# gabrielmpp/LagrangianCoherence

Hardware: AMD Instinct MI355X
Metric: particle-timesteps/sec (+ FTLE Mcells/sec) at 4096^2 seeds per GPU (higher is better)
Workload: dtype f32

## Files before the change

### include/lcs_hip.h

```cpp
#ifndef LCS_HIP_H
#define LCS_HIP_H

#include <stddef.h>
#include <stdint.h>

#ifdef __cplusplus
extern "C" {
#endif

#define LC_VERSION 104

typedef struct lc_ctx lc_ctx;

enum lc_dtype {
    LC_F32 = 0,
    LC_F64 = 1,
    LC_F64_WIND_F32 = 2,
    LC_F64_WIND_F32_LIN32 = 3
};

enum lc_status {
    LC_OK = 0,
    LC_EINVAL = -1,
    LC_EUNSUPPORTED = -2,
// ... 11 lines not shown
enum lc_tensor_layout {
    LC_LAYOUT_REFERENCE = 0,
    LC_LAYOUT_PHYSICAL = 1
};

int lc_version(void);
const char *lc_last_error(void);
const char *lc_build_id(void);

int lc_ctx_create(int device, lc_ctx **out);
int lc_ctx_destroy(lc_ctx *ctx);
int lc_ctx_set_stream(lc_ctx *ctx, void *hip_stream );
int lc_ctx_use_own_stream(lc_ctx *ctx);
int lc_sync(lc_ctx *ctx);

int lc_ctx_set_lds_tiles(lc_ctx *ctx, int mode);
int lc_ctx_set_sigma_march(lc_ctx *ctx, int on);
typedef int (*lc_flag_allreduce_fn)(void *user, void *flags_dev, size_t count);
int lc_ctx_set_flag_allreduce(lc_ctx *ctx, lc_flag_allreduce_fn fn, void *user);
int lc_ctx_set_level_chunk(lc_ctx *ctx, int levels);
int lc_ctx_get_level_chunk(const lc_ctx *ctx, int *levels_out);
int lc_ctx_set_level_grading(lc_ctx *ctx, int chunk, int zone, int depth);
int lc_ctx_get_level_grading(const lc_ctx *ctx, int *chunk_out, int *zone_out, int *depth_out);
enum lc_f64_fidelity { LC_F64_AUTO = 0, LC_F64_EXACT_ORDER = 1, LC_F64_FAST = 2 };
#define LC_EXACT_ORDER_MAX_SEEDS (1 << 18)
int lc_ctx_set_f64_fidelity(lc_ctx *ctx, int mode);
int lc_ctx_get_f64_fidelity(const lc_ctx *ctx, int *mode_out);
int lc_ctx_set_host_pipeline(lc_ctx *ctx, int on);
int lc_copy_to_device(lc_ctx *ctx, void *dst_dev, const void *src_host, size_t bytes);
int lc_copy_to_host(lc_ctx *ctx, void *dst_host, const void *src_dev, size_t bytes);
int lc_ctx_set_host_cache(lc_ctx *ctx, int on);
int lc_ctx_trim(lc_ctx *ctx);
int lc_ctx_last_host_marks(const lc_ctx *ctx, double *ms4_out);
int lc_ctx_set_xcd_split(lc_ctx *ctx, int split);
const char *lc_ctx_last_advect_kernel(const lc_ctx *ctx);
int lc_ctx_last_advect_launches(const lc_ctx *ctx);
const char *lc_ctx_last_sigma_kernel(const lc_ctx *ctx);
const char *lc_ctx_last_pack_kernel(const lc_ctx *ctx);
const char *lc_ctx_last_tracer_kernel(const lc_ctx *ctx);
#define LC_VERIFY_WORDS 16
int lc_ctx_set_verify(lc_ctx *ctx, int mode);
int lc_ctx_read_verify(lc_ctx *ctx, unsigned *out16, int reset);

int lc_malloc(lc_ctx *ctx, size_t bytes, void **dev_out);
int lc_free(lc_ctx *ctx, void *dev);
int lc_memcpy_h2d(lc_ctx *ctx, void *dev_dst, const void *host_src, size_t bytes);
// ... 196 lines not shown
```

### lagrangiancoherence_amd/_capi.py

```python
from __future__ import annotations

import ctypes as C
import os

HERE = os.path.dirname(os.path.abspath(__file__))
LIB_PATH = os.path.join(HERE, "liblcs_hip.so")

LC_VERSION = 104
LC_F32, LC_F64, LC_F64_WIND_F32, LC_F64_WIND_F32_LIN32 = 0, 1, 2, 3
LC_OK, LC_EINVAL, LC_EUNSUPPORTED, LC_EHIP, LC_ENOMEM, LC_ERCCL = 0, -1, -2, -3, -4, -5
LC_LAYOUT_REFERENCE, LC_LAYOUT_PHYSICAL = 0, 1
LC_X_CLAMP_POINT, LC_X_CYCLIC, LC_X_CLAMP_REFERENCE_OUTER = 0, 1, 2
LC_GRID_REGULAR, LC_GRID_GAUSSIAN = 0, 1
LC_F64_AUTO, LC_F64_EXACT_ORDER, LC_F64_FAST = 0, 1, 2
LC_EXACT_ORDER_MAX_SEEDS = 1 << 18

_vp, _i, _d, _sz = C.c_void_p, C.c_int, C.c_double, C.c_size_t

PROTOTYPES = {
    "lc_version": (_i, []),
    "lc_last_error": (C.c_char_p, []),
    "lc_build_id": (C.c_char_p, []),
    "lc_ctx_create": (_i, [_i, C.POINTER(_vp)]),
    "lc_ctx_destroy": (_i, [_vp]),
    "lc_ctx_set_stream": (_i, [_vp, _vp]),
    "lc_ctx_use_own_stream": (_i, [_vp]),
    "lc_sync": (_i, [_vp]),
    "lc_ctx_set_lds_tiles": (_i, [_vp, _i]),
    "lc_ctx_set_sigma_march": (_i, [_vp, _i]),
    "lc_ctx_set_level_chunk": (_i, [_vp, _i]),
    "lc_ctx_get_level_chunk": (_i, [_vp, C.POINTER(_i)]),
    "lc_ctx_set_level_grading": (_i, [_vp, _i, _i, _i]),
    "lc_ctx_get_level_grading": (_i, [_vp, C.POINTER(_i), C.POINTER(_i), C.POINTER(_i)]),
    "lc_ctx_set_f64_fidelity": (_i, [_vp, _i]),
    "lc_ctx_get_f64_fidelity": (_i, [_vp, C.POINTER(_i)]),
    "lc_ctx_set_host_pipeline": (_i, [_vp, _i]),
    "lc_ctx_last_host_marks": (_i, [_vp, C.POINTER(C.c_double)]),
    "lc_copy_to_device": (_i, [_vp, _vp, _vp, C.c_size_t]),
    "lc_copy_to_host": (_i, [_vp, _vp, _vp, C.c_size_t]),
    "lc_ctx_set_host_cache": (_i, [_vp, _i]),
    "lc_ctx_trim": (_i, [_vp]),
    "lc_ctx_set_xcd_split": (_i, [_vp, _i]),
    "lc_ctx_set_flag_allreduce": (_i, [_vp, _vp, _vp]),
    "lc_ctx_last_advect_kernel": (C.c_char_p, [_vp]),
    "lc_ctx_last_advect_launches": (_i, [_vp]),
    "lc_ctx_last_sigma_kernel": (C.c_char_p, [_vp]),
    "lc_ctx_last_pack_kernel": (C.c_char_p, [_vp]),
    "lc_ctx_last_tracer_kernel": (C.c_char_p, [_vp]),
    "lc_ctx_set_verify": (_i, [_vp, _i]),
    "lc_ctx_read_verify": (_i, [_vp, C.POINTER(C.c_uint), _i]),
    "lc_malloc": (_i, [_vp, _sz, C.POINTER(_vp)]),
    "lc_free": (_i, [_vp, _vp]),
    "lc_memcpy_h2d": (_i, [_vp, _vp, _vp, _sz]),
    "lc_memcpy_d2h": (_i, [_vp, _vp, _vp, _sz]),
    "lc_packed_elems": (_sz, [_i, _i, _i]),
    "lc_field_pack": (_i, [_vp, _vp, _vp, _i, _i, _i, _i, _i, _vp, _vp]),
# ... 147 lines not shown
```

### lagrangiancoherence_amd/csrc/advect.hip

```cpp
#include <initializer_list>
#include <type_traits>
#include <vector>

#include "lcs_common.h"
#include "launch_plan.h"

namespace {

constexpr int TILE_W = 8;
constexpr int TILE_H = 32;
constexpr int BLOCK = TILE_W * TILE_H;

template <typename T>
struct AdvectArgs {
    const T *lin;
    const T *img;
    const T *ext;
    const T *u_raw, *v_raw;
    const float *lin32;
    const float *u_raw32, *v_raw32;
    size_t raw_plane;
    int ext_raw;
    int ext_cub;
    size_t level_elems;
// ... 14 lines not shown
    int n_members, member_t0_stride;
    size_t member_plane;
    int pair_d, pair_l0, pair_n, pair_g, pair_last;
    size_t pair_plane;
    int traj_skip0;
    int traj_pair_ok, out_pair_ok;
    int traj_line_ok;
    int patch_mode;
    int xcd_rows;
    int xcd_split;
    int wg64;
    int ntx, ntiles;
    int xcd_chunk;
    int tile_order;
    int tile_order_two_seed;
    int pole_blocks, pole_lo, pole_hi;
    unsigned *clamp_flag;
    int clamp_stride;
    unsigned *verify;
    int member_dirs;
    lcplan::Grading grade;
    int grade_launch, grade_t0;
    const T *grade_x_start, *grade_y_start;
#ifdef LCS_TIMELINE
    unsigned long long *timeline;
    int timeline_launch;
#endif
};

template <typename T>
__device__ __forceinline__ int xcd_tile_id(const AdvectArgs<T> &A) {
    return lcplan::tile_of_block((int)blockIdx.x - A.pole_blocks, A.ntiles, A.ntx, A.xcd_chunk, A.tile_order);
}
template <typename T>
static inline unsigned nmem(const AdvectArgs<T> &A) { return A.n_members > 1 ? (unsigned)A.n_members : 1u; }

template <typename K, typename T, typename... Extra>
static inline const char *launch_kernel(K kernel, int grid, hipStream_t st, const AdvectArgs<T> &A, const char *name, const Extra &...extra) {
    hipLaunchKernelGGL(kernel, dim3(grid, nmem(A)), dim3(BLOCK), 0, st, A, extra...);
    return name;
}

template <typename T>
struct Instance {
    int K;
    bool cyclic;
// ... 1472 lines not shown
#endif
#ifndef LCS_LDS2_DPP_NEXT
#define LCS_LDS2_DPP_NEXT 1
#endif
#ifndef LCS_LDS2_DIRECT_LEVELS
#define LCS_LDS2_DIRECT_LEVELS 0
#endif
template <int KFIX, bool CYCLIC, int MODE>
__global__ void __launch_bounds__(BLOCK, LCS_LDS2_MINWAVES) __attribute__((amdgpu_num_sgpr(LCS_LDS2_NUM_SGPR)))
    advect_lds2_kernel(const AdvectArgs<float> A0) {
#pragma clang fp contract(fast)
    const AdvectArgs<float> A = for_member(A0);
    constexpr bool WIDE = MODE == PATCH_WIDE, LINES = MODE == PATCH_LINES, GROUP = MODE == PATCH_PAIR;
    constexpr int NS = SPL;
    constexpr int ORDER = 1;
    constexpr bool DEFER_X = LCS_LDS2_DEFER_X != 0;
    constexpr int DIRECT_LEVELS = DEFER_X ? LCS_LDS2_DIRECT_LEVELS : 0;
    constexpr bool DPP_NEXT = LCS_LDS2_DPP_NEXT != 0 && 16 % Lds2Geom::LANES_PER_ROW == 0;
    const int K = KFIX >= 0 ? KFIX : A.K;
    typedef Lds2Geom G;
    constexpr int LT_COLS = G::COLS, LT_ROWS = LCS_LDS2_ROWS;
    constexpr int LT_PITCH = LCS_LDS2_PITCH;
    constexpr int WIN = 2, WOFF = LC_PAD_LO;
    __shared__ __attribute__((aligned(16))) f4 s_tiles[BLOCK / 64][LT_ROWS * LT_PITCH];
    __shared__ __attribute__((aligned(16))) float s_slab[2][2][LINES ? 16 * SLAB_PITCH : 4];
    if (GROUP ? pole_block_group(A) : pole_block<float, POLE_LIN>(A)) return;
    int tile_id, t0 = A.t0, nsteps = A.nsteps;
    const float *x_from = A.x_start, *y_from = A.y_start;
    if (MODE == PATCH_TALL && A.grade.n > 0) {
        const int d = (int)blockIdx.x - A.pole_blocks;
        tile_id = lcplan::tile_of_block(lcplan::graded_slot(A.grade, A.grade_launch, d), A.ntiles, A.ntx, A.xcd_chunk, A.tile_order);
        if (tile_id >= A.ntiles) return;
        const lcplan::Range r = lcplan::graded_range(A.grade, A.grade_launch, d);
        if (r.b <= r.a) return;
        t0 = A.grade_t0 + r.a;
        nsteps = r.b - r.a;
        x_from = r.a == 0 ? A.grade_x_start : A.x_out;
        y_from = r.a == 0 ? A.grade_y_start : A.y_out;
    } else {
        tile_id = xcd_tile_id(A);
        if (tile_id >= A.ntiles) return;
    }
    const int tyi = tile_id / A.ntx, txi = tile_id - tyi * A.ntx;
    const int lane = threadIdx.x & 63, wave = threadIdx.x >> 6;
#ifdef LCS_TIMELINE
    unsigned long long *const tl_rec = A.timeline ? A.timeline + ((size_t)A.timeline_launch * gridDim.x + blockIdx.x) * 4 : nullptr;
    if (tl_rec && threadIdx.x == 0) {
// ... 74 lines not shown
    unsigned pitch_bytes = (unsigned)LT_PITCH * 16u;
    asm volatile("" : "+s"(pitch_bytes));
    const f2 pmin = {A.lon_min, A.lat_min}, sc = {A.sx, A.sy};
    auto to_index = [&](f2 v) { return (v - pmin) * sc; };
    const float xlo = A.x_min, xhi = A.x_max;
    auto x_needs_care = [&](float x) { return CYCLIC ? !(fabsf(x) < 180.0f) : !((x > xlo) & (x < xhi)); };
    const float *lvl = A.img + (size_t)t0 * A.level_elems;
    const float *elv = A.ext + (size_t)t0 * A.level_elems;
    const int pad_cols = A.pitch, pad_rows = A.ny_f + LC_PAD;
    const float kpred = 0.5f * (float)(K > 0 ? K - 1 : 0);
    const int st_row = min(lane / G::LANES_PER_ROW, LT_ROWS - 1), st_col = (lane % G::LANES_PER_ROW) * 2;
    const unsigned st_off = ((unsigned)st_row * (unsigned)pad_cols + (unsigned)st_col) * 8u;
    constexpr int NPASS = (LT_ROWS + G::ROWS_PER_PASS - 1) / G::ROWS_PER_PASS;
    const unsigned st_next = st_off + (st_col + 2 < LT_COLS ? 16u : 0u);
    constexpr int CENTRE = (WIDE || GROUP) ? TILE_W / 2 + TILE_W * 4 : TILE_W / 2 + TILE_W * 7;
    f2 dprev = {0.0f, 0.0f};
    const int nlev = GROUP ? lcplan::group_levels(A.nsteps, A.pair_l0, A.pair_n, A.pair_d, cnt) : nsteps;
#ifdef LCS_STAMPS
    long long acc_t[5] = {0, 0, 0, 0, 0}, last_t = __builtin_amdgcn_s_memtime();
    unsigned long long acc_n[3] = {0, 0, 0};
    int prev_redos = 0;
#endif
    int direct_left = 0;
    for (int s = 0; s < nlev; ++s) {
        const bool direct = DIRECT_LEVELS > 0 && direct_left > 0;
        if (direct) --direct_left;
#ifdef LCS_STAMPS
        int level_redos = 0;
#endif
        f2 c0[NS];
#pragma unroll
        for (int q = 0; q < NS; ++q) c0[q] = to_index(p[q]);
        bool act[NS];
        f2 keep[NS];
        int qa = 0;
        if (GROUP) {
            int qlo = NS, qhi = 0;
#pragma unroll
            for (int q = 0; q < NS; ++q) {
                act[q] = lcplan::member_steps(q, s, A.pair_l0, A.pair_n, A.pair_d) && q < cnt;
                keep[q] = p[q];
                if (act[q]) {
                    qlo = min(qlo, q);
                    qhi = q;
                }
            }
            qa = min(max(NS / 2, qlo), qhi);
        }
        auto of_anchor = [&](const f2 (&v)[NS]) {
            f2 r = v[0];
#pragma unroll
            for (int q = 1; q < NS; ++q) r = (GROUP && qa == q) ? v[q] : r;
            return r;
        };
        int ox = 0, oy = 0;
        f4 stage[NPASS];
        f2 stage_next[NPASS];
        if (K > 0 && !direct) {
            const f2 ca = dprev * (1.0f + kpred) + of_anchor(c0);
            const int rxm = __builtin_amdgcn_readlane((int)floor_to_uint(ca.x), CENTRE);
            const int rym = __builtin_amdgcn_readlane((int)floor_to_uint(ca.y), CENTRE);
            ox = min(max(rxm + WOFF - (LT_COLS - WIN) / 2, 0), pad_cols - LT_COLS);
            oy = min(max(rym + WOFF - (LT_ROWS - WIN) / 2, 0), pad_rows - LT_ROWS);
            const char *src = (const char *)elv + ((size_t)__umul24((unsigned)oy, (unsigned)pad_cols) + (unsigned)ox) * 8;
#pragma unroll
            for (int r = 0; r < NPASS; ++r) {
                __builtin_memcpy(&stage[r], src + (size_t)(r * G::ROWS_PER_PASS) * pad_cols * 8 + st_off, 16);
                if (!DPP_NEXT) __builtin_memcpy(&stage_next[r], src + (size_t)(r * G::ROWS_PER_PASS) * pad_cols * 8 + st_next, 8);
            }
        }
        LCS_STAMP(0)
        f2 e[NS], pn[NS];
        bool bad[NS], anybad = false;
#pragma unroll
        for (int q = 0; q < NS; ++q) {
            const TapL t = tap_of(c0[q]);
            bad[q] = ((unsigned)t.x0 > (unsigned)(A.nx_f - 2)) | ((unsigned)t.y0 > (unsigned)(A.ny_f - 2));
            e[q] = euler_global<ORDER>(lvl, A, t);
            pn[q] = dd[q] * e[q] + p[q];
            if (!DEFER_X) bad[q] |= x_needs_care(pn[q].x);
            anybad |= bad[q];
        }
        if (anybad) {
#pragma unroll
            for (int q = 0; q < NS; ++q) {
                if (bad[q]) {
                    const TapL t = tap_of(index_coords(A, p[q]));
                    e[q] = euler_global<ORDER>(lvl, A, t);
                    pn[q] = dd[q] * e[q] + p[q];
                    if (!DEFER_X) clamp_position_p(A, pn[q], ymax_v);
                }
            }
        }
        dprev = (of_anchor(pn) - of_anchor(p)) * sc;
#pragma unroll
        for (int q = 0; q < NS; ++q) p[q] = pn[q];
#ifdef LCS_STAMPS
        asm volatile("" : : "v"(p[0].x), "v"(p[1].x));
#endif
        LCS_STAMP(1)
        int lo_x = 0x40000000, lo_y = 0x40000000, lim_x = 0, lim_y = 0;
        unsigned base_addr = tile_addr;
        if (K > 0 && !direct) {
            __builtin_amdgcn_wave_barrier();
#pragma unroll
            for (int r = 0; r < NPASS; ++r) {
                f2 nxt;
                if constexpr (DPP_NEXT) {
                    float nx0, nx1;
                    const float s0 = stage[r].x, s1 = stage[r].y;
                    asm volatile("s_nop 4\n\tv_mov_b32_dpp %0, %2 row_shl:1 row_mask:0xf bank_mask:0xf bound_ctrl:0\n\t"
                                 "v_mov_b32_dpp %1, %3 row_shl:1 row_mask:0xf bank_mask:0xf bound_ctrl:0"
                                 : "=&v"(nx0), "=&v"(nx1) : "v"(s0), "v"(s1));
                    nxt = (f2){nx0, nx1};
                } else {
                    nxt = stage_next[r];
                }
                f4 *dst = tile + (r * G::ROWS_PER_PASS + st_row) * LT_PITCH + st_col;
                const f2 n0 = stage[r].xy, n1 = stage[r].zw, d0 = n1 - n0, d1 = nxt - n1;
                dst[0] = (f4){n0.x, n0.y, d0.x, d0.y};
                dst[1] = (f4){n1.x, n1.y, d1.x, d1.y};
            }
            __builtin_amdgcn_wave_barrier();
            const int sox = ox - WOFF, soy = oy - WOFF;
            const int hx = min(sox + LT_COLS - WIN, A.nx_f - 2), hy = min(soy + LT_ROWS - WIN, A.ny_f - 2);
            const int lx = max(sox, DEFER_X ? 1 : 0), ly = max(soy, DEFER_X ? 1 : 0);
            if (hx >= lx && hy >= ly) {
                lo_x = lx;
                lo_y = ly;
                lim_x = hx - lx;
                lim_y = hy - ly;
                base_addr = tile_addr + (unsigned)(lx - sox) * 16u + (unsigned)(ly - soy) * ((unsigned)LT_PITCH * 16u);
            }
        }
#ifdef LCS_STAMPS
        asm volatile("s_waitcnt vmcnt(0) lgkmcnt(0)" ::: "memory");
#endif
        LCS_STAMP(2)
        int redos = 0;
        if (direct) {
#pragma unroll 1
            for (int k = 0; k < K; ++k) {
#pragma unroll
                for (int q = 0; q < NS; ++q) {
                    f2 pc = p[q];
                    clamp_position_c<CYCLIC>(A, pc, ymax_v);
                    const TapL t = tap_of(index_coords(A, pc));
                    p[q] = hd[q] * window_global<ORDER>(elv, A, t, e[q]) + pc;
                }
            }
        } else
#pragma unroll
        for (int k = 0; k < K; ++k) {
            anybad = false;
#pragma unroll
            for (int q = 0; q < NS; ++q) {
                typedef __attribute__((address_space(3))) const f4 lds_f4;
                const TapL t = tap_of(to_index(p[q]));
                const int rx = t.x0 - lo_x, ry = t.y0 - lo_y;
                bad[q] = ((unsigned)rx > (unsigned)lim_x) | ((unsigned)ry > (unsigned)lim_y);
#ifdef LCS_STAMPS
                {
                    const unsigned long long bx = __ballot((unsigned)rx > (unsigned)lim_x), by = __ballot((unsigned)ry > (unsigned)lim_y);
                    const unsigned long long bxl = __ballot(rx < 0), byl = __ballot(ry < 0);
                    if (lane == 0) {
                        atomicAdd(&g_cause[0], (unsigned long long)__popcll(bx));
                        atomicAdd(&g_cause[1], (unsigned long long)__popcll(by));
                        atomicAdd(&g_cause[2], (unsigned long long)__popcll(bxl));
                        atomicAdd(&g_cause[3], (unsigned long long)__popcll(byl));
                    }
                }
#endif
                unsigned row_addr;
                asm("v_mad_u32_u24 %0, %1, %2, %3" : "=v"(row_addr) : "v"(ry), "s"(pitch_bytes), "v"(base_addr));
                lds_f4 *cell = (lds_f4 *)(size_t)(row_addr + ((unsigned)rx << 4));
                const f4 c0 = cell[0], c1 = cell[LT_PITCH];
                const f2 r0 = c0.xy + t.tx * c0.zw;
                const f2 r1 = c1.xy + t.tx * c1.zw;
                const f2 ew = e[q] + (r0 + t.ty * (r1 - r0));
                pn[q] = hd[q] * ew + p[q];
                if (!DEFER_X) bad[q] |= x_needs_care(pn[q].x);
                anybad |= bad[q];
            }
#ifdef LCS_STAMPS
            {
                const unsigned long long m0 = __ballot(bad[0]), m1 = __ballot(bad[1]);
                if (lane == 0) {
                    acc_n[0] += 1;
                    acc_n[1] += (m0 | m1) ? 1 : 0;
                    level_redos += (m0 | m1) ? 1 : 0;
                    acc_n[2] += __popcll(m0) + __popcll(m1);
                    const int band = min(2, (int)(fabsf(A.seed_lat[min(iy0, A.ny - 1)]) / 30.0f)), third = min(2, 3 * s / A.nsteps);
                    atomicAdd(&g_redo[band][third][0], 1ull);
                    atomicAdd(&g_redo[band][third][1], (m0 | m1) ? 1ull : 0ull);
                    atomicAdd(&g_redo[band][third][2], (unsigned long long)(__popcll(m0) + __popcll(m1)));
                }
            }
#endif
            if (DIRECT_LEVELS > 0) redos += __ballot(anybad) != 0ull;
            if (anybad) {
#pragma unroll
                for (int q = 0; q < NS; ++q) {
                    if (bad[q]) {
                        f2 pc = p[q];
                        if (DEFER_X)
                            clamp_position_c<CYCLIC>(A, pc, ymax_v);
                        else
                            pc.y = __builtin_amdgcn_fmed3f(pc.y, A.y_min, ymax_v);
                        const TapL t = tap_of(index_coords(A, pc));
                        pn[q] = hd[q] * window_global<ORDER>(elv, A, t, e[q]) + pc;
                        if (!DEFER_X) clamp_position_p(A, pn[q], ymax_v);
                    }
                }
            }
#pragma unroll
            for (int q = 0; q < NS; ++q) p[q] = pn[q];
        }
        if (DIRECT_LEVELS > 0 && redos >= 3) direct_left = DIRECT_LEVELS;
#pragma unroll
        for (int q = 0; q < NS; ++q) {
            if (DEFER_X)
                clamp_position_c<CYCLIC>(A, p[q], ymax_v);
            else
                p[q].y = __builtin_amdgcn_fmed3f(p[q].y, A.y_min, ymax_v);
        }
        if (GROUP) {
#pragma unroll
            for (int q = 0; q < NS; ++q)
                if (!act[q]) p[q] = keep[q];
        }
        if (LINES && lines) {
            float *sx = s_slab[s & 1][0], *sy = s_slab[s & 1][1];
#pragma unroll
            for (int q = 0; q < NS; ++q) {
                const int o = (lane / TILE_W + 8 * q) * SLAB_PITCH + wave * TILE_W + (lane % TILE_W);
                sx[o] = p[q].x;
                sy[o] = p[q].y;
            }
            asm volatile("s_waitcnt lgkmcnt(0)\n\ts_barrier" ::: "memory");
            const f4 line = *(const f4 *)(s_slab[s & 1][wave >> 1] + sl_row * SLAB_PITCH + sl_col);
            if (sl_ok) {
// ... 14 lines not shown
            prev_redos = level_redos;
        }
#endif
        lvl += A.level_elems;
        elv += A.level_elems;
    }
#ifdef LCS_STAMPS
    if (lane == 0) {
        for (int i = 0; i < 4; ++i) atomicAdd(&g_stamps[i], (unsigned long long)acc_t[i]);
        for (int i = 0; i < 3; ++i) atomicAdd(&g_stamps[4 + i], acc_n[i]);
    }
#endif
    if (WIDE && pair && A.out_pair_ok) {
        *(f2 *)(A.x_out + idx[0]) = (f2){p[0].x, p[1].x};
        *(f2 *)(A.y_out + idx[0]) = (f2){p[0].y, p[1].y};
    } else {
#pragma unroll
        for (int q = 0; q < NS; ++q) {
            if (live[q]) {
                A.x_out[idx[q]] = p[q].x;
                A.y_out[idx[q]] = p[q].y;
            }
        }
    }
#ifdef LCS_TIMELINE
    if (tl_rec && lane == 0) atomicMax(tl_rec + 1, (unsigned long long)wall_clock64());
#endif
}

template <int MODE>
struct PatchLanes {
    static constexpr bool WIDE = MODE == PATCH_WIDE, LINES = MODE == PATCH_LINES;
    bool live[SPL], any, pair, lines, sl_ok;
    f2 p[SPL], dd[SPL], hd[SPL];
    size_t idx[SPL], sl_idx, plane;
    int lane, wave, sl_row, sl_col;

    __device__ __forceinline__ void init(const AdvectArgs<float> &A, int txi, int tyi) {
        lane = threadIdx.x & 63;
        wave = threadIdx.x >> 6;
        plane = (size_t)A.ny * A.nx;
        const int ix0 = WIDE ? txi * (TILE_W * SPL) + SPL * (lane % TILE_W)
                      : LINES ? txi * (TILE_W * 4) + wave * TILE_W + (lane % TILE_W) : txi * TILE_W + (lane % TILE_W);
        const int iy0 = WIDE ? tyi * TILE_H + wave * 8 + lane / TILE_W
                      : LINES ? tyi * (8 * SPL) + lane / TILE_W : tyi * (TILE_H * SPL) + wave * (8 * SPL) + lane / TILE_W;
        any = false;
// ... 1680 lines not shown
    A.xcd_split = ctx->xcd_split;
    set_field_geometry(A, call.src, a);
    A.ext = (order == 1 || order == 3) ? (const T *)call.ext : nullptr;
    A.lin32 = (sizeof(T) == 8 && order == 1) ? (const float *)call.lin32 : nullptr;
    A.u_raw32 = (sizeof(T) == 8 && order == 3) ? (const float *)call.lin32 : nullptr;
    A.v_raw32 = (sizeof(T) == 8 && order == 3) ? (const float *)call.lin32_v : nullptr;
    A.ext_raw = a.fuse_levels_raw && sizeof(T) == 8 && order == 1 && call.src.u_raw && !call.wind_f32 && !call.ext;
    A.ext_cub = a.fuse_levels_raw && sizeof(T) == 8 && order == 3 && call.src.cub && !call.wind_f32 && !call.ext;
    A.y_min = (T)a.lat_min;
    A.y_max = (T)a.lat_max;
    A.x_min = (T)a.lon_min;
    A.x_max = (T)a.lon_max;
    A.seed_lat = (const T *)a.seed_lat_dev;
    A.seed_lon = (const T *)a.seed_lon_dev;
    const double conv_y = 180.0 / (6371000.0 * 3.141592653589793);
    A.dt = (T)a.timestep;
    A.half_dt = (T)(0.5 * a.timestep);
    A.dtcy = (T)(a.timestep * conv_y);
    A.hdtcy = (T)((0.5 * a.timestep) * conv_y);
    A.K = K;
    A.cyclic = a.cyclic_x == LC_X_CYCLIC;
    A.clamp_flag = nullptr;
    A.verify = sizeof(T) == 4 ? ctx->verify_dev : nullptr;
    A.t0 = a.t0;
    A.nsteps = a.nsteps;
    A.x_out = (T *)a.x_out;
    A.y_out = (T *)a.y_out;
    A.traj_x = (T *)a.traj_x;
    A.traj_y = (T *)a.traj_y;
    A.ntx = (nx + TILE_W - 1) / TILE_W;
    const int nty = (ny + TILE_H - 1) / TILE_H;
    A.ntiles = A.ntx * nty;
    A.xcd_chunk = lcplan::xcd_chunk_tiles(A.ntx, nty, ctx->xcd_chunk_rows, ctx->xcd_split);
    A.wg64 = ctx->f64_wg_tile;
    A.tile_order = ctx->tile_order >= 0 ? ctx->tile_order : 1;
    A.tile_order_two_seed = ctx->tile_order >= 0 ? ctx->tile_order : 2;
    {
        const lcplan::PoleRows pr = lcplan::pole_rows(A.order, A.row0, ny, A.ny_global, nx, ctx->pole_blocks != 0, BLOCK);
        A.pole_lo = pr.lo;
        A.pole_hi = pr.hi;
        A.pole_blocks = pr.blocks;
    }
    return A;
}

template <typename T>
// ... 662 lines not shown
```

### lagrangiancoherence_amd/csrc/api.hip

```cpp
#include <chrono>
#include <cmath>
#include <cstdlib>
#include <cstring>
#include <vector>

#include "hostxfer.h"
#include "lcs_common.h"

static thread_local char g_err[1024] = "";

void lc_set_error(const char *fmt, ...) {
    va_list ap;
    va_start(ap, fmt);
    vsnprintf(g_err, sizeof(g_err), fmt, ap);
    va_end(ap);
}

extern "C" const char *lc_last_error(void) { return g_err; }
extern "C" int lc_version(void) { return LC_VERSION; }
#ifndef LCS_BUILD_ID
#define LCS_BUILD_ID "unstamped"
#endif
extern "C" const char *lc_build_id(void) { return LCS_BUILD_ID; }

// ... 25 lines not shown
        else (void)hipGetLastError();
    }
    c->lds_tiles = 3;
    if (const char *ev = getenv("LCS_LDS_TILES")) c->lds_tiles = ev[0] == '0' ? 0 : (ev[0] == '2' ? 2 : (ev[0] == '1' ? 1 : 3));
    c->xcd_chunk_rows = 1;
    if (const char *ev = getenv("LCS_XCD_CHUNK_ROWS")) c->xcd_chunk_rows = atoi(ev) > 0 ? atoi(ev) : 0;
    c->xcd_split = -1;
    if (const char *ev = getenv("LCS_XCD_SPLIT")) c->xcd_split = atoi(ev) >= 0 ? atoi(ev) : -1;
    c->tile_order = -1;
    if (const char *ev = getenv("LCS_TILE_ORDER")) c->tile_order = (ev[0] >= '0' && ev[0] <= '3') ? ev[0] - '0' : -1;
    c->pole_blocks = 1;
    if (const char *ev = getenv("LCS_POLE_BLOCKS")) c->pole_blocks = ev[0] != '0';
    c->fir_prefilter = 1;
    if (const char *ev = getenv("LCS_FIR_PREFILTER")) c->fir_prefilter = ev[0] == '0' ? 0 : (ev[0] == '2' ? 2 : 1);
    c->fused_prefilter = 1;
    if (const char *ev = getenv("LCS_FUSED_PREFILTER")) c->fused_prefilter = ev[0] != '0';
    c->sigma_march = 2;
    if (const char *ev = getenv("LCS_SIGMA_MARCH")) c->sigma_march = ev[0] == '0' ? 0 : (ev[0] == '1' ? 1 : 2);
    c->level_chunk = -1;
    if (const char *ev = getenv("LCS_LEVEL_CHUNK")) c->level_chunk = atoi(ev) >= 0 ? atoi(ev) : -1;
    c->grade_chunk = 0;
    c->grade_zone = -1;
    c->grade_depth = -1;
#ifdef LCS_TIMELINE
    c->timeline_dev = nullptr;
    c->timeline_cap = 0;
    c->timeline_launches = c->timeline_grid = 0;
#endif
    c->f64_fidelity = LC_F64_AUTO;
    if (const char *ev = getenv("LCS_F64_FIDELITY")) c->f64_fidelity = ev[0] == 'e' ? LC_F64_EXACT_ORDER : (ev[0] == 'f' ? LC_F64_FAST : LC_F64_AUTO);
    c->patch_mode = -1;
    if (const char *ev = getenv("LCS_PATCH_MODE")) c->patch_mode = (ev[0] >= '0' && ev[0] <= '3') ? ev[0] - '0' : -1;
    c->flag_reduce = nullptr;
    c->flag_reduce_user = nullptr;
    c->lds_tiles_init = c->lds_tiles;
    c->sigma_march_init = c->sigma_march;
    c->last_advect_kernel = "";
    c->last_advect_launches = 0;
    c->last_sigma_kernel = "";
    c->last_pack_kernel = "";
    c->last_tracer_kernel = "";
    c->last_strain_kernel = "";
    c->verify_dev = nullptr;
    c->trunc = nullptr;
    c->xfer = nullptr;
    c->host_ws = nullptr;
// ... 78 lines not shown
    LC_REQUIRE(levels >= -1, "lc_ctx_set_level_chunk: levels must be >= -1 (0 = one launch for the whole series, -1 = by size)");
    ctx->level_chunk = levels;
    return LC_OK;
}

extern "C" int lc_ctx_set_level_grading(lc_ctx *ctx, int chunk, int zone, int depth) {
    LC_REQUIRE(ctx, "lc_ctx_set_level_grading: null context");
    LC_REQUIRE(chunk >= 0 && zone >= -1 && depth >= -1,
               "lc_ctx_set_level_grading: chunk must be >= 0 (0 = by size), zone and depth >= -1 (-1 = the default; depth 0 = off)");
    ctx->grade_chunk = chunk;
    ctx->grade_zone = zone;
    ctx->grade_depth = depth;
    return LC_OK;
}

extern "C" int lc_ctx_get_level_grading(const lc_ctx *ctx, int *chunk_out, int *zone_out, int *depth_out) {
    LC_REQUIRE(ctx && chunk_out && zone_out && depth_out, "lc_ctx_get_level_grading: null pointer");
    *chunk_out = ctx->grade_chunk;
    *zone_out = ctx->grade_zone;
    *depth_out = ctx->grade_depth;
    return LC_OK;
}

extern "C" int lc_ctx_set_verify(lc_ctx *ctx, int mode) {
    LC_REQUIRE(ctx, "lc_ctx_set_verify: null context");
    LC_REQUIRE(mode >= 0 && mode <= 2, "lc_ctx_set_verify: mode must be 0 (off), 1 (audit) or 2 (audit + one injected corruption)");
    LC_HIP_CHECK(hipSetDevice(ctx->device));
    LC_HIP_CHECK(hipStreamSynchronize(ctx->stream));
    if (mode == 0) {
        if (ctx->verify_dev) LC_HIP_CHECK(hipFree(ctx->verify_dev));
        ctx->verify_dev = nullptr;
        return LC_OK;
    }
    if (!ctx->verify_dev) {
        hipError_t e = hipMalloc((void **)&ctx->verify_dev, LC_VERIFY_WORDS * sizeof(unsigned));
        if (e != hipSuccess) {
            ctx->verify_dev = nullptr;
            (void)hipGetLastError();
            lc_set_error("lc_ctx_set_verify: hipMalloc failed: %s", hipGetErrorString(e));
            return e == hipErrorOutOfMemory ? LC_ENOMEM : LC_EHIP;
        }
    }
    unsigned init[LC_VERIFY_WORDS] = {};
    init[15] = mode == 2 ? 0xBADu : 0u;
    LC_HIP_CHECK(hipMemcpy(ctx->verify_dev, init, sizeof(init), hipMemcpyHostToDevice));
    return LC_OK;
// ... 9 lines not shown
        unsigned init[LC_VERIFY_WORDS] = {};
        init[15] = out16[15];
        LC_HIP_CHECK(hipMemcpy(ctx->verify_dev, init, sizeof(init), hipMemcpyHostToDevice));
    }
    return LC_OK;
}

extern "C" const char *lc_ctx_last_advect_kernel(const lc_ctx *ctx) { return ctx ? ctx->last_advect_kernel : ""; }
extern "C" int lc_ctx_last_advect_launches(const lc_ctx *ctx) { return ctx ? ctx->last_advect_launches : 0; }
extern "C" const char *lc_ctx_last_sigma_kernel(const lc_ctx *ctx) { return ctx ? ctx->last_sigma_kernel : ""; }
extern "C" const char *lc_ctx_last_pack_kernel(const lc_ctx *ctx) { return ctx ? ctx->last_pack_kernel : ""; }
extern "C" const char *lc_ctx_last_tracer_kernel(const lc_ctx *ctx) { return ctx ? ctx->last_tracer_kernel : ""; }

static void host_ws_destroy(lc_ctx *ctx);

extern "C" int lc_ctx_destroy(lc_ctx *ctx) {
    if (!ctx) return LC_OK;
    (void)hipSetDevice(ctx->device);
    (void)hipStreamSynchronize(ctx->stream);
    lc_trunc_cache_free(ctx->trunc);
    lc_host_xfer::release(ctx->xfer);
    host_ws_destroy(ctx);
    if (ctx->verify_dev) (void)hipFree(ctx->verify_dev);
#ifdef LCS_TIMELINE
    if (ctx->timeline_dev) (void)hipFree(ctx->timeline_dev);
#endif
    (void)hipStreamDestroy(ctx->own_stream);
    delete ctx;
    return LC_OK;
}

extern "C" int lc_ctx_set_stream(lc_ctx *ctx, void *hip_stream) {
    LC_REQUIRE(ctx, "lc_ctx_set_stream: null context");
    ctx->stream = (hipStream_t)hip_stream;
    return LC_OK;
}

extern "C" int lc_ctx_use_own_stream(lc_ctx *ctx) {
    LC_REQUIRE(ctx, "lc_ctx_use_own_stream: null context");
    ctx->stream = ctx->own_stream;
    return LC_OK;
}

extern "C" int lc_sync(lc_ctx *ctx) {
    LC_REQUIRE(ctx, "lc_sync: null context");
    LC_HIP_CHECK(hipSetDevice(ctx->device));
// ... 661 lines not shown
```

### lagrangiancoherence_amd/csrc/lcs_common.h

```cpp
#pragma once
#include <hip/hip_runtime.h>

#include <cstdarg>
#include <cstdio>

#include "../../include/lcs_hip.h"

struct lc_trunc_cache;
void lc_trunc_cache_free(lc_trunc_cache *c);

struct lc_ctx {
    int device;
    int n_cus;
    hipStream_t own_stream;
    hipStream_t stream;
    int lds_tiles;
    int lds_tiles_init, sigma_march_init;
    int sigma_march;
    int xcd_split;
    int xcd_chunk_rows;
    int fir_prefilter;
    int fused_prefilter;
    int tile_order;
    int pole_blocks;
    int level_chunk;
    int f64_fidelity;
    int patch_mode;
    lc_flag_allreduce_fn flag_reduce;
    void *flag_reduce_user;
    int last_advect_launches;
    const char *last_advect_kernel;
    const char *last_sigma_kernel;
    const char *last_pack_kernel;
    const char *last_tracer_kernel;
    unsigned *verify_dev;
    lc_trunc_cache *trunc;
    struct lc_host_xfer *xfer;
    void *host_ws;
    int host_cache;
    double host_marks[4];
    int host_timing;
    int f64_wg_tile;
    int host_threads;
    int host_piece_mb;
    int host_pipeline;
    const char *last_strain_kernel;
    int grade_chunk, grade_zone, grade_depth;
#ifdef LCS_TIMELINE
    unsigned long long *timeline_dev;
    size_t timeline_cap;
    int timeline_launches, timeline_grid;
#endif
};

void lc_set_error(const char *fmt, ...);

#define LC_HIP_CHECK(expr)                                                              \
    do {                                                                                \
        hipError_t _e = (expr);                                                         \
        if (_e != hipSuccess) {                                                         \
            lc_set_error("%s failed: %s (%s:%d)", #expr, hipGetErrorString(_e), __FILE__, \
                         __LINE__);                                                     \
            (void)hipGetLastError();                                                    \
            return LC_EHIP;                                                             \
        }                                                                               \
    } while (0)

#define LC_REQUIRE(cond, ...)          \
    do {                               \
        if (!(cond)) {                 \
// ... 65 lines not shown
```

### lagrangiancoherence_amd/engine.py

```python
from __future__ import annotations

import ctypes as C
import os
from collections import namedtuple
from dataclasses import dataclass

import numpy as np

from . import _capi

__all__ = ["Engine", "PackedField", "PackedTracer", "lcs_host", "lcs_global_host", "common_dtype", "x_boundary_mode"]

_NP2LC = {np.dtype(np.float32): _capi.LC_F32, np.dtype(np.float64): _capi.LC_F64}
_LAYOUTS = {"reference": _capi.LC_LAYOUT_REFERENCE, "physical": _capi.LC_LAYOUT_PHYSICAL}


def x_boundary_mode(cyclic_xboundary, noncyclic_clamp=None, whole_grid=True) -> int:
    if cyclic_xboundary:
        return _capi.LC_X_CYCLIC
    if noncyclic_clamp is None:
        noncyclic_clamp = "reference_outer"
    if noncyclic_clamp not in ("pointwise", "reference_outer"):
        raise ValueError(f"noncyclic_clamp {noncyclic_clamp!r}: 'pointwise' or 'reference_outer'")
    return _capi.LC_X_CLAMP_REFERENCE_OUTER if noncyclic_clamp == "reference_outer" else _capi.LC_X_CLAMP_POINT
# ... 153 lines not shown
        _capi.check(self.lib.lc_ctx_set_lds_tiles(self.ctx, int(mode)), self.lib)
        self.lds_tiles_mode = int(mode)

    def set_sigma_march(self, on: int):
        _capi.check(self.lib.lc_ctx_set_sigma_march(self.ctx, int(on)), self.lib)

    def set_level_chunk(self, levels: int):
        _capi.check(self.lib.lc_ctx_set_level_chunk(self.ctx, int(levels)), self.lib)

    @property
    def level_chunk(self) -> int:
        v = C.c_int()
        _capi.check(self.lib.lc_ctx_get_level_chunk(self.ctx, C.byref(v)), self.lib)
        return v.value

    def set_level_grading(self, chunk: int = 0, zone: int = -1, depth: int = -1):
        _capi.check(self.lib.lc_ctx_set_level_grading(self.ctx, int(chunk), int(zone), int(depth)), self.lib)

    @property
    def level_grading(self):
        c, z, d = C.c_int(), C.c_int(), C.c_int()
        _capi.check(self.lib.lc_ctx_get_level_grading(self.ctx, C.byref(c), C.byref(z), C.byref(d)), self.lib)
        return c.value, z.value, d.value

    _FIDELITY = {"auto": _capi.LC_F64_AUTO, "exact": _capi.LC_F64_EXACT_ORDER, "fast": _capi.LC_F64_FAST}

    def set_f64_fidelity(self, mode: str):
        if mode not in self._FIDELITY:
            raise ValueError(f"float64 fidelity {mode!r}: 'auto', 'exact' or 'fast'")
        _capi.check(self.lib.lc_ctx_set_f64_fidelity(self.ctx, self._FIDELITY[mode]), self.lib)

    def f64_fuse_levels(self, dtype, n_seeds: int) -> bool:
        if np.dtype(dtype) != np.dtype(np.float64):
            return True
        m = C.c_int()
        _capi.check(self.lib.lc_ctx_get_f64_fidelity(self.ctx, C.byref(m)), self.lib)
        if m.value == _capi.LC_F64_EXACT_ORDER:
            return False
        return m.value == _capi.LC_F64_FAST or int(n_seeds) > _capi.LC_EXACT_ORDER_MAX_SEEDS

    def set_flag_allreduce(self, group=None, comm=None, enable=True):
        if not enable:
            _capi.check(self.lib.lc_ctx_set_flag_allreduce(self.ctx, None, None), self.lib)
            self._flag_cb = None
            return
        if comm is not None:
# ... 990 lines not shown
```

Before: 254.0 billion.

## Adaptively double LDS tile height after redo iterations in tall-patch advection

Adds an adaptive mode to the LDS2 advection kernel. After a level in which a wave hit a redo (tap out of the staged tile), the staged LDS tile height doubles for a held number of levels. Each iteration now tracks a redo mask with ballots, and the extra staged rows use an additional load and LDS store. The intent is to cut costly redo/fallback paths for fast-moving particles, at the cost of doubled LDS allocation (lower occupancy risk), extra VGPRs and extra staging traffic on tall levels.

```diff
diff --git a/include/lcs_hip.h b/include/lcs_hip.h
--- a/include/lcs_hip.h
+++ b/include/lcs_hip.h
@@ -57,6 +57,15 @@
 int lc_ctx_get_level_chunk(const lc_ctx *ctx, int *levels_out);
 int lc_ctx_set_level_grading(lc_ctx *ctx, int chunk, int zone, int depth);
 int lc_ctx_get_level_grading(const lc_ctx *ctx, int *chunk_out, int *zone_out, int *depth_out);
+enum lc_tall_tiles { LC_TALL_TILES_NEVER = 0, LC_TALL_TILES_ADAPTIVE = 1, LC_TALL_TILES_ALWAYS = 2 };
+#define LC_TALL_TILES_MAX_TRIGGER 4
+#define LC_TALL_TILES_DEFAULT_MODE LC_TALL_TILES_ADAPTIVE
+#define LC_TALL_TILES_DEFAULT_TRIGGER 1
+#define LC_TALL_TILES_DEFAULT_HOLD 8
+int lc_ctx_set_tall_tiles(lc_ctx *ctx, int mode, int trigger, int hold);
+int lc_ctx_get_tall_tiles(const lc_ctx *ctx, int *mode_out, int *trigger_out, int *hold_out);
+int lc_ctx_count_tall_tiles(lc_ctx *ctx, int on);
+int lc_ctx_read_tall_tiles(lc_ctx *ctx, unsigned long long *out2, int reset);
 enum lc_f64_fidelity { LC_F64_AUTO = 0, LC_F64_EXACT_ORDER = 1, LC_F64_FAST = 2 };
 #define LC_EXACT_ORDER_MAX_SEEDS (1 << 18)
 int lc_ctx_set_f64_fidelity(lc_ctx *ctx, int mode);
diff --git a/lagrangiancoherence_amd/_capi.py b/lagrangiancoherence_amd/_capi.py
--- a/lagrangiancoherence_amd/_capi.py
+++ b/lagrangiancoherence_amd/_capi.py
@@ -32,6 +32,10 @@
     "lc_ctx_get_level_chunk": (_i, [_vp, C.POINTER(_i)]),
     "lc_ctx_set_level_grading": (_i, [_vp, _i, _i, _i]),
     "lc_ctx_get_level_grading": (_i, [_vp, C.POINTER(_i), C.POINTER(_i), C.POINTER(_i)]),
+    "lc_ctx_set_tall_tiles": (_i, [_vp, _i, _i, _i]),
+    "lc_ctx_get_tall_tiles": (_i, [_vp, C.POINTER(_i), C.POINTER(_i), C.POINTER(_i)]),
+    "lc_ctx_count_tall_tiles": (_i, [_vp, _i]),
+    "lc_ctx_read_tall_tiles": (_i, [_vp, C.POINTER(C.c_ulonglong), _i]),
     "lc_ctx_set_f64_fidelity": (_i, [_vp, _i]),
     "lc_ctx_get_f64_fidelity": (_i, [_vp, C.POINTER(_i)]),
     "lc_ctx_set_host_pipeline": (_i, [_vp, _i]),
diff --git a/lagrangiancoherence_amd/csrc/advect.hip b/lagrangiancoherence_amd/csrc/advect.hip
--- a/lagrangiancoherence_amd/csrc/advect.hip
+++ b/lagrangiancoherence_amd/csrc/advect.hip
@@ -60,6 +60,8 @@
     lcplan::Grading grade;
     int grade_launch, grade_t0;
     const T *grade_x_start, *grade_y_start;
+    int tall_mode, tall_trigger, tall_hold;
+    unsigned long long *tall_count;
 #ifdef LCS_TIMELINE
     unsigned long long *timeline;
     int timeline_launch;
@@ -1578,7 +1580,9 @@
     constexpr int LT_COLS = G::COLS, LT_ROWS = LCS_LDS2_ROWS;
     constexpr int LT_PITCH = LCS_LDS2_PITCH;
     constexpr int WIN = 2, WOFF = LC_PAD_LO;
-    __shared__ __attribute__((aligned(16))) f4 s_tiles[BLOCK / 64][LT_ROWS * LT_PITCH];
+    constexpr bool TALLK = MODE == PATCH_TALL && KFIX != 0 && DPP_NEXT && LT_ROWS == G::ROWS_PER_PASS;
+    constexpr int LT_ROWS_MAX = TALLK ? 2 * LT_ROWS : LT_ROWS;
+    __shared__ __attribute__((aligned(16))) f4 s_tiles[BLOCK / 64][LT_ROWS_MAX * LT_PITCH];
     __shared__ __attribute__((aligned(16))) float s_slab[2][2][LINES ? 16 * SLAB_PITCH : 4];
     if (GROUP ? pole_block_group(A) : pole_block<float, POLE_LIN>(A)) return;
     int tile_id, t0 = A.t0, nsteps = A.nsteps;
@@ -1699,9 +1703,13 @@
     int prev_redos = 0;
 #endif
     int direct_left = 0;
+    const int tall_trig = TALLK && A.tall_mode == 1 ? A.tall_trigger : 0x7fffffff, tall_set = TALLK && A.tall_mode == 1 ? A.tall_hold : 0;
+    const int tall_min = TALLK && A.tall_mode == 2 ? 1 : 0;
+    int hold = tall_min, row_sum = 0;
     for (int s = 0; s < nlev; ++s) {
         const bool direct = DIRECT_LEVELS > 0 && direct_left > 0;
         if (direct) --direct_left;
+        const int rows = TALLK && hold > 0 ? LT_ROWS_MAX : LT_ROWS;
 #ifdef LCS_STAMPS
         int level_redos = 0;
 #endif
@@ -1733,18 +1741,20 @@
         int ox = 0, oy = 0;
         f4 stage[NPASS];
         f2 stage_next[NPASS];
+        f4 stage_hi;
         if (K > 0 && !direct) {
             const f2 ca = dprev * (1.0f + kpred) + of_anchor(c0);
             const int rxm = __builtin_amdgcn_readlane((int)floor_to_uint(ca.x), CENTRE);
             const int rym = __builtin_amdgcn_readlane((int)floor_to_uint(ca.y), CENTRE);
             ox = min(max(rxm + WOFF - (LT_COLS - WIN) / 2, 0), pad_cols - LT_COLS);
-            oy = min(max(rym + WOFF - (LT_ROWS - WIN) / 2, 0), pad_rows - LT_ROWS);
+            oy = min(max(rym + WOFF - (rows - WIN) / 2, 0), pad_rows - rows);
             const char *src = (const char *)elv + ((size_t)__umul24((unsigned)oy, (unsigned)pad_cols) + (unsigned)ox) * 8;
 #pragma unroll
             for (int r = 0; r < NPASS; ++r) {
                 __builtin_memcpy(&stage[r], src + (size_t)(r * G::ROWS_PER_PASS) * pad_cols * 8 + st_off, 16);
                 if (!DPP_NEXT) __builtin_memcpy(&stage_next[r], src + (size_t)(r * G::ROWS_PER_PASS) * pad_cols * 8 + st_next, 8);
             }
+            if (TALLK && rows > LT_ROWS) __builtin_memcpy(&stage_hi, src + (size_t)LT_ROWS * pad_cols * 8 + st_off, 16);
         }
         LCS_STAMP(0)
         f2 e[NS], pn[NS];
@@ -1780,27 +1790,29 @@
         unsigned base_addr = tile_addr;
         if (K > 0 && !direct) {
             __builtin_amdgcn_wave_barrier();
-#pragma unroll
-            for (int r = 0; r < NPASS; ++r) {
+            auto stage_pass = [&](const f4 &sv, const f2 &sv_next, int row0) {
                 f2 nxt;
                 if constexpr (DPP_NEXT) {
                     float nx0, nx1;
-                    const float s0 = stage[r].x, s1 = stage[r].y;
+                    const float s0 = sv.x, s1 = sv.y;
                     asm volatile("s_nop 4\n\tv_mov_b32_dpp %0, %2 row_shl:1 row_mask:0xf bank_mask:0xf bound_ctrl:0\n\t"
                                  "v_mov_b32_dpp %1, %3 row_shl:1 row_mask:0xf bank_mask:0xf bound_ctrl:0"
                                  : "=&v"(nx0), "=&v"(nx1) : "v"(s0), "v"(s1));
                     nxt = (f2){nx0, nx1};
                 } else {
-                    nxt = stage_next[r];
+                    nxt = sv_next;
                 }
-                f4 *dst = tile + (r * G::ROWS_PER_PASS + st_row) * LT_PITCH + st_col;
-                const f2 n0 = stage[r].xy, n1 = stage[r].zw, d0 = n1 - n0, d1 = nxt - n1;
+                f4 *dst = tile + (row0 + st_row) * LT_PITCH + st_col;
+                const f2 n0 = sv.xy, n1 = sv.zw, d0 = n1 - n0, d1 = nxt - n1;
                 dst[0] = (f4){n0.x, n0.y, d0.x, d0.y};
                 dst[1] = (f4){n1.x, n1.y, d1.x, d1.y};
-            }
+            };
+#pragma unroll
+            for (int r = 0; r < NPASS; ++r) stage_pass(stage[r], stage_next[r], r * G::ROWS_PER_PASS);
+            if (TALLK && rows > LT_ROWS) stage_pass(stage_hi, stage_next[0], LT_ROWS);
             __builtin_amdgcn_wave_barrier();
             const int sox = ox - WOFF, soy = oy - WOFF;
-            const int hx = min(sox + LT_COLS - WIN, A.nx_f - 2), hy = min(soy + LT_ROWS - WIN, A.ny_f - 2);
+            const int hx = min(sox + LT_COLS - WIN, A.nx_f - 2), hy = min(soy + rows - WIN, A.ny_f - 2);
             const int lx = max(sox, DEFER_X ? 1 : 0), ly = max(soy, DEFER_X ? 1 : 0);
             if (hx >= lx && hy >= ly) {
                 lo_x = lx;
@@ -1830,12 +1842,14 @@
 #pragma unroll
         for (int k = 0; k < K; ++k) {
             anybad = false;
+            unsigned long long redo_mask = 0ull;
 #pragma unroll
             for (int q = 0; q < NS; ++q) {
                 typedef __attribute__((address_space(3))) const f4 lds_f4;
                 const TapL t = tap_of(to_index(p[q]));
                 const int rx = t.x0 - lo_x, ry = t.y0 - lo_y;
                 bad[q] = ((unsigned)rx > (unsigned)lim_x) | ((unsigned)ry > (unsigned)lim_y);
+                if (TALLK) redo_mask |= __builtin_amdgcn_ballot_w64((unsigned)rx > (unsigned)lim_x) | __builtin_amdgcn_ballot_w64((unsigned)ry > (unsigned)lim_y);
 #ifdef LCS_STAMPS
                 {
                     const unsigned long long bx = __ballot((unsigned)rx > (unsigned)lim_x), by = __ballot((unsigned)ry > (unsigned)lim_y);
@@ -1857,6 +1871,7 @@
                 const f2 ew = e[q] + (r0 + t.ty * (r1 - r0));
                 pn[q] = hd[q] * ew + p[q];
                 if (!DEFER_X) bad[q] |= x_needs_care(pn[q].x);
+                if (!DEFER_X && TALLK) redo_mask |= __builtin_amdgcn_ballot_w64(x_needs_care(pn[q].x));
                 anybad |= bad[q];
             }
 #ifdef LCS_STAMPS
@@ -1874,7 +1889,8 @@
                 }
             }
 #endif
-            if (DIRECT_LEVELS > 0) redos += __ballot(anybad) != 0ull;
+            if (DIRECT_LEVELS > 0 && !TALLK) redos += __ballot(anybad) != 0ull;
+            if (TALLK) asm volatile("s_cmp_lg_u64 %1, 0\n\ts_addc_u32 %0, %0, 0" : "+s"(redos) : "s"(redo_mask) : "scc");
             if (anybad) {
 #pragma unroll
                 for (int q = 0; q < NS; ++q) {
@@ -1894,6 +1910,10 @@
             for (int q = 0; q < NS; ++q) p[q] = pn[q];
         }
         if (DIRECT_LEVELS > 0 && redos >= 3) direct_left = DIRECT_LEVELS;
+        if (TALLK) {
+            row_sum += rows;
+            hold = redos >= tall_trig ? tall_set : max(hold - 1, tall_min);
+        }
 #pragma unroll
         for (int q = 0; q < NS; ++q) {
             if (DEFER_X)
@@ -1954,6 +1974,10 @@
                 A.y_out[idx[q]] = p[q].y;
             }
         }
+    }
+    if (TALLK && A.tall_count && lane == 0) {
+        atomicAdd(A.tall_count, (unsigned long long)((row_sum - nlev * LT_ROWS) / (LT_ROWS_MAX - LT_ROWS)));
+        atomicAdd(A.tall_count + 1, (unsigned long long)nlev);
     }
 #ifdef LCS_TIMELINE
     if (tl_rec && lane == 0) atomicMax(tl_rec + 1, (unsigned long long)wall_clock64());
@@ -3680,6 +3704,10 @@
     A.cyclic = a.cyclic_x == LC_X_CYCLIC;
     A.clamp_flag = nullptr;
     A.verify = sizeof(T) == 4 ? ctx->verify_dev : nullptr;
+    A.tall_mode = ctx->tall_mode;
+    A.tall_trigger = ctx->tall_trigger;
+    A.tall_hold = ctx->tall_hold;
+    A.tall_count = ctx->tall_count_dev;
     A.t0 = a.t0;
     A.nsteps = a.nsteps;
     A.x_out = (T *)a.x_out;
diff --git a/lagrangiancoherence_amd/csrc/api.hip b/lagrangiancoherence_amd/csrc/api.hip
--- a/lagrangiancoherence_amd/csrc/api.hip
+++ b/lagrangiancoherence_amd/csrc/api.hip
@@ -71,6 +71,13 @@
     c->grade_chunk = 0;
     c->grade_zone = -1;
     c->grade_depth = -1;
+#ifndef LCS_TALL_TILES_MODE
+#define LCS_TALL_TILES_MODE LC_TALL_TILES_DEFAULT_MODE
+#endif
+    c->tall_mode = LCS_TALL_TILES_MODE;
+    c->tall_trigger = LC_TALL_TILES_DEFAULT_TRIGGER;
+    c->tall_hold = LC_TALL_TILES_DEFAULT_HOLD;
+    c->tall_count_dev = nullptr;
 #ifdef LCS_TIMELINE
     c->timeline_dev = nullptr;
     c->timeline_cap = 0;
@@ -195,6 +202,63 @@
     return LC_OK;
 }
 
+extern "C" int lc_ctx_set_tall_tiles(lc_ctx *ctx, int mode, int trigger, int hold) {
+    LC_REQUIRE(ctx, "lc_ctx_set_tall_tiles: null context");
+    LC_REQUIRE(mode >= LC_TALL_TILES_NEVER && mode <= LC_TALL_TILES_ALWAYS, "lc_ctx_set_tall_tiles: mode must be 0 (never), 1 (adaptive) or 2 (always)");
+    LC_REQUIRE(trigger >= 1 && trigger <= LC_TALL_TILES_MAX_TRIGGER, "lc_ctx_set_tall_tiles: trigger must be 1 .. %d iterations with a redo",
+               LC_TALL_TILES_MAX_TRIGGER);
+    LC_REQUIRE(hold >= 1, "lc_ctx_set_tall_tiles: hold must be >= 1 level");
+    ctx->tall_mode = mode;
+    ctx->tall_trigger = trigger;
+    ctx->tall_hold = hold;
+    return LC_OK;
+}
+
+extern "C" int lc_ctx_get_tall_tiles(const lc_ctx *ctx, int *mode_out, int *trigger_out, int *hold_out) {
+    LC_REQUIRE(ctx && mode_out && trigger_out && hold_out, "lc_ctx_get_tall_tiles: null pointer");
+    *mode_out = ctx->tall_mode;
+    *trigger_out = ctx->tall_trigger;
+    *hold_out = ctx->tall_hold;
+    return LC_OK;
+}
+
+extern "C" int lc_ctx_count_tall_tiles(lc_ctx *ctx, int on) {
+    LC_REQUIRE(ctx, "lc_ctx_count_tall_tiles: null context");
+    LC_REQUIRE(on == 0 || on == 1, "lc_ctx_count_tall_tiles: 0 or 1");
+    LC_HIP_CHECK(hipSetDevice(ctx->device));
+    LC_HIP_CHECK(hipStreamSynchronize(ctx->stream));
+    if (!on) {
+        if (ctx->tall_count_dev) LC_HIP_CHECK(hipFree(ctx->tall_count_dev));
+        ctx->tall_count_dev = nullptr;
+        return LC_OK;
+    }
+    if (!ctx->tall_count_dev) {
+        hipError_t e = hipMalloc((void **)&ctx->tall_count_dev, 2 * sizeof(unsigned long long));
+        if (e != hipSuccess) {
+            ctx->tall_count_dev = nullptr;
+            (void)hipGetLastError();
+            lc_set_error("lc_ctx_count_tall_tiles: hipMalloc failed: %s", hipGetErrorString(e));
+            return e == hipErrorOutOfMemory ? LC_ENOMEM : LC_EHIP;
+        }
+    }
+    const unsigned long long zero[2] = {0ull, 0ull};
+    LC_HIP_CHECK(hipMemcpy(ctx->tall_count_dev, zero, sizeof(zero), hipMemcpyHostToDevice));
+    return LC_OK;
+}
+
+extern "C" int lc_ctx_read_tall_tiles(lc_ctx *ctx, unsigned long long *out2, int reset) {
+    LC_REQUIRE(ctx && out2, "lc_ctx_read_tall_tiles: null pointer");
+    LC_REQUIRE(ctx->tall_count_dev, "lc_ctx_read_tall_tiles: the count is off (lc_ctx_count_tall_tiles)");
+    LC_HIP_CHECK(hipSetDevice(ctx->device));
+    LC_HIP_CHECK(hipStreamSynchronize(ctx->stream));
+    LC_HIP_CHECK(hipMemcpy(out2, ctx->tall_count_dev, 2 * sizeof(unsigned long long), hipMemcpyDeviceToHost));
+    if (reset) {
+        const unsigned long long zero[2] = {0ull, 0ull};
+        LC_HIP_CHECK(hipMemcpy(ctx->tall_count_dev, zero, sizeof(zero), hipMemcpyHostToDevice));
+    }
+    return LC_OK;
+}
+
 extern "C" int lc_ctx_set_verify(lc_ctx *ctx, int mode) {
     LC_REQUIRE(ctx, "lc_ctx_set_verify: null context");
     LC_REQUIRE(mode >= 0 && mode <= 2, "lc_ctx_set_verify: mode must be 0 (off), 1 (audit) or 2 (audit + one injected corruption)");
@@ -250,6 +314,7 @@
     lc_host_xfer::release(ctx->xfer);
     host_ws_destroy(ctx);
     if (ctx->verify_dev) (void)hipFree(ctx->verify_dev);
+    if (ctx->tall_count_dev) (void)hipFree(ctx->tall_count_dev);
 #ifdef LCS_TIMELINE
     if (ctx->timeline_dev) (void)hipFree(ctx->timeline_dev);
 #endif
diff --git a/lagrangiancoherence_amd/csrc/lcs_common.h b/lagrangiancoherence_amd/csrc/lcs_common.h
--- a/lagrangiancoherence_amd/csrc/lcs_common.h
+++ b/lagrangiancoherence_amd/csrc/lcs_common.h
@@ -46,6 +46,8 @@
     int host_pipeline;
     const char *last_strain_kernel;
     int grade_chunk, grade_zone, grade_depth;
+    int tall_mode, tall_trigger, tall_hold;
+    unsigned long long *tall_count_dev;
 #ifdef LCS_TIMELINE
     unsigned long long *timeline_dev;
     size_t timeline_cap;
diff --git a/lagrangiancoherence_amd/engine.py b/lagrangiancoherence_amd/engine.py
--- a/lagrangiancoherence_amd/engine.py
+++ b/lagrangiancoherence_amd/engine.py
@@ -199,6 +199,23 @@
         c, z, d = C.c_int(), C.c_int(), C.c_int()
         _capi.check(self.lib.lc_ctx_get_level_grading(self.ctx, C.byref(c), C.byref(z), C.byref(d)), self.lib)
         return c.value, z.value, d.value
+
+    def set_tall_tiles(self, mode: int = 1, trigger: int = 1, hold: int = 8):
+        _capi.check(self.lib.lc_ctx_set_tall_tiles(self.ctx, int(mode), int(trigger), int(hold)), self.lib)
+
+    @property
+    def tall_tiles(self):
+        m, t, h = C.c_int(), C.c_int(), C.c_int()
+        _capi.check(self.lib.lc_ctx_get_tall_tiles(self.ctx, C.byref(m), C.byref(t), C.byref(h)), self.lib)
+        return m.value, t.value, h.value
+
+    def count_tall_tiles(self, on: bool = True):
+        _capi.check(self.lib.lc_ctx_count_tall_tiles(self.ctx, int(bool(on))), self.lib)
+
+    def read_tall_tiles(self, reset: bool = True):
+        out = (C.c_ulonglong * 2)()
+        _capi.check(self.lib.lc_ctx_read_tall_tiles(self.ctx, out, int(bool(reset))), self.lib)
+        return int(out[0]), int(out[1])
 
     _FIDELITY = {"auto": _capi.LC_F64_AUTO, "exact": _capi.LC_F64_EXACT_ORDER, "fast": _capi.LC_F64_FAST}
 
```

Result: slower. 249.5 billion (-1.8%).
